# Mephisto405/WCMC

Hardware: AMD Instinct MI355X
Metric: 128x128 MC patches/sec (train step), KPCN-Manifold (higher is better)
Workload: dtype bf16x321h

## Files before the change

### wcmc_amd/csrc/pathnet_fused.hip

```cpp
#include <stdlib.h>

#include "common.h"

namespace wcmc {

typedef __bf16 bf16x8 __attribute__((ext_vector_type(8)));
typedef unsigned short u16;
typedef short s16x4 __attribute__((ext_vector_type(4)));
typedef unsigned u32x2 __attribute__((ext_vector_type(2)));
typedef unsigned u32x4 __attribute__((ext_vector_type(4)));

constexpr unsigned E3_OOB = 0x80000000u;
constexpr int E3_TP = 64;
constexpr int E3_C = 64;
constexpr int E3_RS = 80;
constexpr int E3_TILE = E3_TP * E3_RS;

__device__ __forceinline__ u16 e3_bf(float x) { return __builtin_bit_cast(u16, (__bf16)x); }
__device__ __forceinline__ float e3_f(u16 h) { return __builtin_bit_cast(float, (unsigned)h << 16); }
__device__ __forceinline__ float e3_u2f(unsigned v) { return __builtin_bit_cast(float, v); }
__device__ __forceinline__ unsigned e3_f2u(float v) { return __builtin_bit_cast(unsigned, v); }

struct E3Params {
  const u16* x; int64_t M; int Cp0, Kt0;
// ... 196 lines not shown
                                                                       p.gm ? (int)p.gm_bytes : 0, 0x00020000);
  const E3W w0 = e3_load_w(p.wp0, 16 * ct + fr, q, p.Kt0), w1 = e3_load_w(p.wp1, 16 * ct + fr, q);
  const E3W t2 = e3_load_w(p.wt2, 16 * ct + fr, q), t1 = e3_load_w(p.wt1, 16 * ct + fr, q);
  float b0[4], b1[4];
#pragma unroll
  for (int e = 0; e < 4; ++e) { const int co = 16 * ct + 4 * q + e; b0[e] = p.b0[co]; b1[e] = p.b1[co]; }
  f32x4 g2[2], g1[2], g0[2];
#pragma unroll
  for (int j = 0; j < 2; ++j) { g2[j] = f32x4{0.f, 0.f, 0.f, 0.f}; g1[j] = g2[j]; g0[j] = g2[j]; }
  const int nci0 = (p.Cp0 + 15) >> 4;
  float sb2[4] = {0.f, 0.f, 0.f, 0.f}, sb1[4] = {0.f, 0.f, 0.f, 0.f}, sb0[4] = {0.f, 0.f, 0.f, 0.f};
  const int64_t ntiles = (p.M + E3_TP - 1) / E3_TP;
  const int64_t SHW = (int64_t)p.S * p.HW;

  struct DyPre { u32x4 g[2], m[2]; };
  const bool mean_uniform = p.HW % E3_TP == 0;
  auto load_dy = [&](int64_t m0) {
    DyPre r;
    const unsigned gbase = (unsigned)(m0 * p.gy_ps * 4);
    const int left = (int)(p.M - m0 < E3_TP ? p.M - m0 : E3_TP);
    const int64_t b = m0 / SHW, hw0 = m0 % p.HW;
    const unsigned mbase = (unsigned)((b * p.HW + hw0) * p.gm_ps * 4);
#pragma unroll
    for (int k = 0; k < 2; ++k) {
      const int v = tid + 512 * k, px = v >> 4, c4 = (v & 15) * 4;
      const bool ok = px < left;
      r.g[k] = __builtin_amdgcn_raw_buffer_load_b128(gyr, ok ? gbase + (unsigned)((px * p.gy_ps + c4) * 4) : E3_OOB, 0, 0);
      unsigned moff;
      if (mean_uniform) {
        moff = mbase + (unsigned)((px * p.gm_ps + c4) * 4);
      } else {
        const unsigned m = (unsigned)m0 + (unsigned)px, bi = m / (unsigned)SHW, hw = m % (unsigned)p.HW;
        moff = (bi * (unsigned)p.HW + hw) * (unsigned)(p.gm_ps * 4) + (unsigned)(c4 * 4);
      }
      r.m[k] = __builtin_amdgcn_raw_buffer_load_b128(gmr, (ok && p.gm) ? moff : E3_OOB, 0, 0);
    }
    return r;
  };
  int64_t t = blockIdx.x;
  E3XPre<512> pre;
  DyPre dpre;
  if (t < ntiles) { pre = e3_load_x<512>(xr, t * E3_TP, p.M, p.Cp0, tid); dpre = load_dy(t * E3_TP); }
  for (; t < ntiles; t += gridDim.x) {
    e3_store_x<512>(pre, XH, XL, tid);
#pragma unroll
    for (int k = 0; k < 2; ++k) {
      const int v = tid + 512 * k, px = v >> 4, c4 = (v & 15) * 4;
      u16 hi[4];
#pragma unroll
      for (int e = 0; e < 4; ++e) {
        const float d = e3_u2f(dpre.g[k][e]) + e3_u2f(dpre.m[k][e]) * p.gm_scale;
        sb2[e] += d;
        hi[e] = e3_bf(d);
      }
      *reinterpret_cast<u32x2*>(DYH + px * E3_RS + c4) = u32x2{(unsigned)hi[0] | ((unsigned)hi[1] << 16), (unsigned)hi[2] | ((unsigned)hi[3] << 16)};
    }
    const int64_t tn = t + gridDim.x;
    if (tn < ntiles) { pre = e3_load_x<512>(xr, tn * E3_TP, p.M, p.Cp0, tid); dpre = load_dy(tn * E3_TP); }
    __syncthreads();
    f32x4 acc[2], acca[2];
    unsigned m0bits = 0;
    e3_gemm<3, 2>(acc, w0, XH, XL, pt0, fr, q);
    e3_gemm<2, 2>(acca, t2, DYH, nullptr, pt0, fr, q);
#pragma unroll
    for (int i = 0; i < 2; ++i) {
      u16 hi[4], lo[4];
#pragma unroll
      for (int e = 0; e < 4; ++e) {
        const float t_ = acc[i][e] + b0[e];
        const float v = t_ > 0.f ? t_ : 0.f;
        hi[e] = e3_bf(v);
        lo[e] = e3_bf(v - e3_f(hi[e]));
        m0bits |= (e3_f(hi[e]) > 0.f ? 1u : 0u) << (4 * i + e);
      }
      const int o = (16 * (pt0 + i) + fr) * E3_RS + 16 * ct + 4 * q;
      *reinterpret_cast<u32x2*>(H0H + o) = u32x2{(unsigned)hi[0] | ((unsigned)hi[1] << 16), (unsigned)hi[2] | ((unsigned)hi[3] << 16)};
      *reinterpret_cast<u32x2*>(H0L + o) = u32x2{(unsigned)lo[0] | ((unsigned)lo[1] << 16), (unsigned)lo[2] | ((unsigned)lo[3] << 16)};
    }
    __syncthreads();
    e3_gemm<3, 2>(acc, w1, H0H, H0L, pt0, fr, q);
#pragma unroll
    for (int i = 0; i < 2; ++i) {
      u16 hi[4], dh[4];
#pragma unroll
      for (int e = 0; e < 4; ++e) {
        const float t_ = acc[i][e] + b1[e];
        hi[e] = e3_bf(t_ > 0.f ? t_ : 0.f);
        const float d = e3_f(hi[e]) > 0.f ? acca[i][e] : 0.f;
        sb1[e] += d;
        dh[e] = e3_bf(d);
      }
      const int o = (16 * (pt0 + i) + fr) * E3_RS + 16 * ct + 4 * q;
      *reinterpret_cast<u32x2*>(H1H + o) = u32x2{(unsigned)hi[0] | ((unsigned)hi[1] << 16), (unsigned)hi[2] | ((unsigned)hi[3] << 16)};
      *reinterpret_cast<u32x2*>(DH1H + o) = u32x2{(unsigned)dh[0] | ((unsigned)dh[1] << 16), (unsigned)dh[2] | ((unsigned)dh[3] << 16)};
    }
    __syncthreads();
    e3_gemm<2, 2>(acc, t1, DH1H, nullptr, pt0, fr, q);
#pragma unroll
    for (int i = 0; i < 2; ++i) {
      u16 dh[4];
#pragma unroll
      for (int e = 0; e < 4; ++e) {
        const float d = ((m0bits >> (4 * i + e)) & 1u) ? acc[i][e] : 0.f;
        sb0[e] += d;
        dh[e] = e3_bf(d);
      }
      const int o = (16 * (pt0 + i) + fr) * E3_RS + 16 * ct + 4 * q;
      *reinterpret_cast<u32x2*>(DH0H + o) = u32x2{(unsigned)dh[0] | ((unsigned)dh[1] << 16), (unsigned)dh[2] | ((unsigned)dh[3] << 16)};
    }
    __syncthreads();
#pragma unroll
    for (int kk = 0; kk < 2; ++kk) {
      const bf16x8 a2 = e3_tr(DYH, kk, ct, lane), a1 = e3_tr(DH1H, kk, ct, lane), a0 = e3_tr(DH0H, kk, ct, lane);
#pragma unroll
      for (int jj = 0; jj < 2; ++jj) {
        const int j = pt0 + jj;
        const bf16x8 bh1 = e3_tr(H1H, kk, j, lane), bh0 = e3_tr(H0H, kk, j, lane);
        g2[jj] = __builtin_amdgcn_mfma_f32_16x16x32_bf16(a2, bh1, g2[jj], 0, 0, 0);
        g1[jj] = __builtin_amdgcn_mfma_f32_16x16x32_bf16(a1, bh0, g1[jj], 0, 0, 0);
        if (j < nci0) {
          const bf16x8 bx = e3_tr(XH, kk, j, lane);
          g0[jj] = __builtin_amdgcn_mfma_f32_16x16x32_bf16(a0, bx, g0[jj], 0, 0, 0);
        }
      }
    }
    __syncthreads();
  }
  float* ws = p.ws + (int64_t)blockIdx.x * E3_WS_PER_BLOCK;
#pragma unroll
  for (int jj = 0; jj < 2; ++jj)
#pragma unroll
    for (int e = 0; e < 4; ++e) {
      const int co = 16 * ct + 4 * q + e, j = pt0 + jj, ci = 16 * j + fr;
      ws[(0 * E3_C + co) * E3_C + ci] = g2[jj][e];
      ws[(1 * E3_C + co) * E3_C + ci] = g1[jj][e];
      ws[(2 * E3_C + co) * E3_C + ci] = j < nci0 ? g0[jj][e] : 0.f;
    }
#pragma unroll
  for (int e = 0; e < 4; ++e) {
    red[0][tid >> 4][(tid & 15) * 4 + e] = sb2[e];
    red[1][16 * ph + fr][16 * ct + 4 * q + e] = sb1[e];
    red[2][16 * ph + fr][16 * ct + 4 * q + e] = sb0[e];
  }
  __syncthreads();
  if (tid < 3 * E3_C) {
    const int l = tid / E3_C, c = tid - l * E3_C;
    float s = 0.f;
#pragma unroll
    for (int r = 0; r < 32; ++r) s += red[l][r][c];
    ws[3 * E3_C * E3_C + l * E3_C + c] = s;
  }
}

__global__ __launch_bounds__(256) void embed3_bwd_finish_kernel(const float* __restrict__ ws, int nblk, int Cin0, float* __restrict__ dw0,
                                                                float* __restrict__ db0, float* __restrict__ dw1, float* __restrict__ db1,
                                                                float* __restrict__ dw2, float* __restrict__ db2) {
  const int i = blockIdx.x * 256 + threadIdx.x;
  if (i >= E3_WS_PER_BLOCK) return;
  float a[8] = {0.f, 0.f, 0.f, 0.f, 0.f, 0.f, 0.f, 0.f};
  int b = 0;
  for (; b + 8 <= nblk; b += 8) {
#pragma unroll
    for (int u = 0; u < 8; ++u) a[u] += ws[(int64_t)(b + u) * E3_WS_PER_BLOCK + i];
  }
  for (; b < nblk; ++b) a[0] += ws[(int64_t)b * E3_WS_PER_BLOCK + i];
  const float s = ((a[0] + a[1]) + (a[2] + a[3])) + ((a[4] + a[5]) + (a[6] + a[7]));
  if (i < 3 * E3_C * E3_C) {
    const int l = i / (E3_C * E3_C), r = i - l * E3_C * E3_C, co = r / E3_C, ci = r - co * E3_C;
    if (l == 0) dw2[co * E3_C + ci] = s;
    else if (l == 1) dw1[co * E3_C + ci] = s;
    else if (ci < Cin0) dw0[co * Cin0 + ci] = s;
  } else {
    const int r = i - 3 * E3_C * E3_C, l = r / E3_C, c = r - l * E3_C;
    (l == 0 ? db2 : l == 1 ? db1 : db0)[c] = s;
  }
}

constexpr int F2_C = 128;
constexpr int F2_RS = 144;
constexpr int F2_TILE = E3_TP * F2_RS;
constexpr int F2_ORS = 48;
constexpr int F2_W1RS = 2 * 128 + 8;

struct F2Params {
  const float* y; int y_ps;
  const float* prop; int p_ps;
  int B, S; int64_t HW;
  const u16* wp0; const u16* wp1;
  const float* b0; const float* b1; int outc;
  float* out; int os;
  const u16* wt0; const u16* wt1;
  const float* gout;
  float* dy; float* dprop;
  float* ws;
  unsigned y_bytes, p_bytes, o_bytes, dy_bytes, dp_bytes;
};
constexpr int F2_WS_PER_BLOCK = F2_C * F2_C + 16 * F2_C + F2_C + 16;

struct F2W { bf16x8 h[4], l[4]; };
__device__ __forceinline__ F2W f2_load_w(const u16* wp, int row, int q) {
  F2W w;
#pragma unroll
  for (int c = 0; c < 4; ++c) {
    const u16* a = wp + (int64_t)(row * 2) * F2_C + c * 32 + q * 8;
    w.h[c] = *reinterpret_cast<const bf16x8*>(a);
    w.l[c] = *reinterpret_cast<const bf16x8*>(a + F2_C);
  }
  return w;
}
template <int TERMS, int NPT>
__device__ __forceinline__ void f2_gemm(f32x4 (&acc)[NPT], const F2W& w, const u16* th, const u16* tl, int pt0, int fr, int q) {
#pragma unroll
  for (int i = 0; i < NPT; ++i) {
    acc[i] = f32x4{0.f, 0.f, 0.f, 0.f};
#pragma unroll
    for (int c = 0; c < 4; ++c) {
      const int o = (16 * (pt0 + i) + fr) * F2_RS + c * 32 + q * 8;
      const bf16x8 ah = *reinterpret_cast<const bf16x8*>(th + o);
      acc[i] = __builtin_amdgcn_mfma_f32_16x16x32_bf16(w.l[c], ah, acc[i], 0, 0, 0);
      if (TERMS == 3) {
        const bf16x8 al = *reinterpret_cast<const bf16x8*>(tl + o);
        acc[i] = __builtin_amdgcn_mfma_f32_16x16x32_bf16(w.h[c], al, acc[i], 0, 0, 0);
      }
      acc[i] = __builtin_amdgcn_mfma_f32_16x16x32_bf16(w.h[c], ah, acc[i], 0, 0, 0);
    }
  }
}
__device__ __forceinline__ bf16x8 f2_tr(const u16* tile, int rs, int kk, int ct, int lane) {
  const int g = lane >> 4, li = lane & 15, tq = li >> 2, tp = li & 3;
  const u16* a0 = tile + (kk * 32 + 4 * g + tq) * rs + ct * 16 + 4 * tp;
  const s16x4 lo4 = __builtin_amdgcn_ds_read_tr16_b64_v4i16((s16x4 __attribute__((address_space(3)))*)(a0));
  const s16x4 hi4 = __builtin_amdgcn_ds_read_tr16_b64_v4i16((s16x4 __attribute__((address_space(3)))*)(a0 + 16 * rs));
  typedef short s16x8 __attribute__((ext_vector_type(8)));
  const s16x8 cat = {lo4[0], lo4[1], lo4[2], lo4[3], hi4[0], hi4[1], hi4[2], hi4[3]};
  return __builtin_bit_cast(bf16x8, cat);
}
struct F2Pre { u32x4 v[2]; };
__device__ __forceinline__ F2Pre f2_load64(const __amdgpu_buffer_rsrc_t r, int64_t m0, int ps, int tid) {
  F2Pre o;
  const unsigned base = (unsigned)(m0 * ps * 4);
#pragma unroll
  for (int k = 0; k < 2; ++k) {
    const int v = tid + 512 * k, px = v >> 4, c4 = (v & 15) * 4;
    o.v[k] = __builtin_amdgcn_raw_buffer_load_b128(r, base + (unsigned)((px * ps + c4) * 4), 0, 0);
  }
  return o;
}
__device__ __forceinline__ void f2_store64_split(const F2Pre& o, u16* th, u16* tl, int c0, int tid) {
#pragma unroll
  for (int k = 0; k < 2; ++k) {
    const int v = tid + 512 * k, px = v >> 4, c4 = (v & 15) * 4;
    u16 hi[4], lo[4];
#pragma unroll
    for (int e = 0; e < 4; ++e) {
      const float f = e3_u2f(o.v[k][e]);
      hi[e] = e3_bf(f);
      lo[e] = e3_bf(f - e3_f(hi[e]));
    }
    const int a = px * F2_RS + c0 + c4;
    *reinterpret_cast<u32x2*>(th + a) = u32x2{(unsigned)hi[0] | ((unsigned)hi[1] << 16), (unsigned)hi[2] | ((unsigned)hi[3] << 16)};
    *reinterpret_cast<u32x2*>(tl + a) = u32x2{(unsigned)lo[0] | ((unsigned)lo[1] << 16), (unsigned)lo[2] | ((unsigned)lo[3] << 16)};
  }
}
__device__ __forceinline__ void f2_store_relu_split(const f32x4 (&acc)[4], const float (&b)[4], u16* th, u16* tl, int wave, int fr, int q) {
#pragma unroll
  for (int i = 0; i < 4; ++i) {
    u16 hi[4], lo[4];
#pragma unroll
    for (int e = 0; e < 4; ++e) {
      const float t = acc[i][e] + b[e];
      const float v = t > 0.f ? t : 0.f;
      hi[e] = e3_bf(v);
      lo[e] = e3_bf(v - e3_f(hi[e]));
    }
    const int o = (16 * i + fr) * F2_RS + 16 * wave + 4 * q;
    *reinterpret_cast<u32x2*>(th + o) = u32x2{(unsigned)hi[0] | ((unsigned)hi[1] << 16), (unsigned)hi[2] | ((unsigned)hi[3] << 16)};
    *reinterpret_cast<u32x2*>(tl + o) = u32x2{(unsigned)lo[0] | ((unsigned)lo[1] << 16), (unsigned)lo[2] | ((unsigned)lo[3] << 16)};
  }
}

template <bool BWD>
__global__ __launch_bounds__(512, 1) void final2_kernel(F2Params p) {
  extern __shared__ __attribute__((aligned(16))) u16 lds[];
  u16* const CH = lds; u16* const CL = lds + F2_TILE; u16* const HH = lds + 2 * F2_TILE; u16* const HL = lds + 3 * F2_TILE;
  u16* const DHH = lds + 4 * F2_TILE;
  u16* const DOH = lds + 5 * F2_TILE;
  float* const stg = reinterpret_cast<float*>(HL);
  float* const red = reinterpret_cast<float*>(lds + 5 * F2_TILE + E3_TP * F2_ORS);
  const int tid = threadIdx.x, lane = tid & 63, wave = tid >> 6, fr = lane & 15, q = lane >> 4;
  const __amdgpu_buffer_rsrc_t yr = __builtin_amdgcn_make_buffer_rsrc((void*)p.y, 0, (int)p.y_bytes, 0x00020000);
  const __amdgpu_buffer_rsrc_t pr = __builtin_amdgcn_make_buffer_rsrc((void*)p.prop, 0, (int)p.p_bytes, 0x00020000);
  const __amdgpu_buffer_rsrc_t orr = __builtin_amdgcn_make_buffer_rsrc((void*)(BWD ? (void*)p.gout : (void*)p.out), 0, (int)p.o_bytes, 0x00020000);
  u16* const W1S = reinterpret_cast<u16*>(red + 16 * F2_C + 64 * 8);
  const F2W w0 = f2_load_w(p.wp0, 16 * wave + fr, q);
  F2W w1;
  if (!BWD) w1 = f2_load_w(p.wp1, fr, q);
  float b0[4], b1[4];
#pragma unroll
  for (int e = 0; e < 4; ++e) { b0[e] = p.b0[16 * wave + 4 * q + e]; b1[e] = (4 * q + e < p.outc) ? p.b1[4 * q + e] : 0.f; }
  const int oq = p.os >> 2;
  const int64_t tpi = p.HW / E3_TP;
  const int64_t nsuper = (int64_t)p.B * tpi;

  F2W t0;
  bf16x8 t1h, t1l;
  f32x4 gw0[8], gw1;
  float sb0[4] = {0.f, 0.f, 0.f, 0.f}, sb1[4] = {0.f, 0.f, 0.f, 0.f};
  __amdgpu_buffer_rsrc_t dyr = yr, dpr = yr;
  if (BWD) {
    t0 = f2_load_w(p.wt0, 16 * wave + fr, q);
    const u16* a = p.wt1 + (int64_t)((16 * wave + fr) * 2) * 32 + q * 8;
    t1h = *reinterpret_cast<const bf16x8*>(a); t1l = *reinterpret_cast<const bf16x8*>(a + 32);
#pragma unroll
    for (int j = 0; j < 8; ++j) gw0[j] = f32x4{0.f, 0.f, 0.f, 0.f};
    gw1 = f32x4{0.f, 0.f, 0.f, 0.f};
    dyr = __builtin_amdgcn_make_buffer_rsrc((void*)p.dy, 0, (int)p.dy_bytes, 0x00020000);
    dpr = __builtin_amdgcn_make_buffer_rsrc((void*)p.dprop, 0, (int)p.dp_bytes, 0x00020000);
    for (int i = tid; i < E3_TP * F2_ORS / 2; i += 512) reinterpret_cast<unsigned*>(DOH)[i] = 0u;
    *reinterpret_cast<u32x4*>(W1S + (tid >> 5) * F2_W1RS + (tid & 31) * 8) = *reinterpret_cast<const u32x4*>(p.wp1 + tid * 8);
  }

  for (int64_t st = blockIdx.x; st < nsuper; st += gridDim.x) {
    const int64_t b = st / tpi, hw0 = (st - b * tpi) * E3_TP;
    F2Pre pp = f2_load64(pr, b * p.HW + hw0, p.p_ps, tid);
    F2Pre yp = f2_load64(yr, (b * p.S) * p.HW + hw0, p.y_ps, tid);
    __syncthreads();
    f2_store64_split(pp, CH, CL, 64, tid);
    f32x4 dpacc[4];
#pragma unroll
    for (int i = 0; i < 4; ++i) dpacc[i] = f32x4{0.f, 0.f, 0.f, 0.f};
    for (int s = 0; s < p.S; ++s) {
      const int64_t m0 = (b * p.S + s) * p.HW + hw0;
      f2_store64_split(yp, CH, CL, 0, tid);
      u32x4 go = {0u, 0u, 0u, 0u};
      if (BWD && wave < 4 && q < oq)
        go = __builtin_amdgcn_raw_buffer_load_b128(orr, (unsigned)(m0 * p.os * 4) + (unsigned)((16 * wave + fr) * p.os * 4 + q * 16), 0, 0);
      if (s + 1 < p.S) yp = f2_load64(yr, (b * p.S + s + 1) * p.HW + hw0, p.y_ps, tid);
      __syncthreads();
      f32x4 acc[4];
      f2_gemm<3, 4>(acc, w0, CH, CL, 0, fr, q);
      f2_store_relu_split(acc, b0, HH, HL, wave, fr, q);
      __syncthreads();
      float ov[4] = {0.f, 0.f, 0.f, 0.f};
      if (wave < 4) {
        f32x4 a2[1];
        if (BWD) {
          a2[0] = f32x4{0.f, 0.f, 0.f, 0.f};
#pragma unroll
          for (int c = 0; c < 4; ++c) {
            const int o = (16 * wave + fr) * F2_RS + c * 32 + q * 8;
            const bf16x8 ah = *reinterpret_cast<const bf16x8*>(HH + o), al = *reinterpret_cast<const bf16x8*>(HL + o);
            const bf16x8 wh = *reinterpret_cast<const bf16x8*>(W1S + fr * F2_W1RS + c * 32 + q * 8);
            const bf16x8 wl = *reinterpret_cast<const bf16x8*>(W1S + fr * F2_W1RS + F2_C + c * 32 + q * 8);
            a2[0] = __builtin_amdgcn_mfma_f32_16x16x32_bf16(wl, ah, a2[0], 0, 0, 0);
            a2[0] = __builtin_amdgcn_mfma_f32_16x16x32_bf16(wh, al, a2[0], 0, 0, 0);
            a2[0] = __builtin_amdgcn_mfma_f32_16x16x32_bf16(wh, ah, a2[0], 0, 0, 0);
          }
        } else {
          f2_gemm<3, 1>(a2, w1, HH, HL, wave, fr, q);
        }
#pragma unroll
        for (int e = 0; e < 4; ++e) { const float t = a2[0][e] + b1[e]; ov[e] = (4 * q + e < p.outc && t > 0.f) ? t : 0.f; }
      }
      if (!BWD) {
        if (wave < 4 && q < oq) {
          const u32x4 o4 = {__builtin_bit_cast(unsigned, ov[0]), __builtin_bit_cast(unsigned, ov[1]), __builtin_bit_cast(unsigned, ov[2]),
                            __builtin_bit_cast(unsigned, ov[3])};
          __builtin_amdgcn_raw_buffer_store_b128(o4, orr, (unsigned)(m0 * p.os * 4) + (unsigned)((16 * wave + fr) * p.os * 4 + q * 16), 0, 0);
        }
        __syncthreads();
        continue;
      }
      if (wave < 4 && q < oq) {
        const int px = 16 * wave + fr;
        u16 hi[4];
#pragma unroll
        for (int e = 0; e < 4; ++e) {
          const float d = ov[e] > 0.f ? e3_u2f(go[e]) : 0.f;
          sb1[e] += d;
          hi[e] = e3_bf(d);
        }
        *reinterpret_cast<u32x2*>(DOH + px * F2_ORS + 4 * q) = u32x2{(unsigned)hi[0] | ((unsigned)hi[1] << 16), (unsigned)hi[2] | ((unsigned)hi[3] << 16)};
      }
      __syncthreads();
#pragma unroll
      for (int i = 0; i < 4; ++i) {
        const bf16x8 dof = *reinterpret_cast<const bf16x8*>(DOH + (16 * i + fr) * F2_ORS + q * 8);
        f32x4 a = f32x4{0.f, 0.f, 0.f, 0.f};
        a = __builtin_amdgcn_mfma_f32_16x16x32_bf16(t1l, dof, a, 0, 0, 0);
        a = __builtin_amdgcn_mfma_f32_16x16x32_bf16(t1h, dof, a, 0, 0, 0);
        const int o = (16 * i + fr) * F2_RS + 16 * wave + 4 * q;
        const u32x2 hm = *reinterpret_cast<const u32x2*>(HH + o);
        u16 hi[4];
#pragma unroll
        for (int e = 0; e < 4; ++e) {
          const u16 hv = (u16)((e < 2 ? hm[0] : hm[1]) >> (16 * (e & 1)));
          const float d = e3_f(hv) > 0.f ? a[e] : 0.f;
          sb0[e] += d;
          hi[e] = e3_bf(d);
        }
        *reinterpret_cast<u32x2*>(DHH + o) = u32x2{(unsigned)hi[0] | ((unsigned)hi[1] << 16), (unsigned)hi[2] | ((unsigned)hi[3] << 16)};
      }
      __syncthreads();
      f2_gemm<2, 4>(acc, t0, DHH, nullptr, 0, fr, q);
      if (wave < 4) {
#pragma unroll
        for (int i = 0; i < 4; ++i)
          *reinterpret_cast<float4*>(stg + (16 * i + fr) * 68 + 16 * wave + 4 * q) = make_float4(acc[i][0], acc[i][1], acc[i][2], acc[i][3]);
      } else {
#pragma unroll
        for (int i = 0; i < 4; ++i) dpacc[i] += acc[i];
      }
#pragma unroll
      for (int kk = 0; kk < 2; ++kk) {
        const bf16x8 a0 = f2_tr(DHH, F2_RS, kk, wave, lane);
#pragma unroll
        for (int j = 0; j < 8; ++j) gw0[j] = __builtin_amdgcn_mfma_f32_16x16x32_bf16(a0, f2_tr(CH, F2_RS, kk, j, lane), gw0[j], 0, 0, 0);
        gw1 = __builtin_amdgcn_mfma_f32_16x16x32_bf16(f2_tr(DOH, F2_ORS, kk, 0, lane), f2_tr(HH, F2_RS, kk, wave, lane), gw1, 0, 0, 0);
      }
      __syncthreads();
#pragma unroll
      for (int k = 0; k < 2; ++k) {
        const int v = tid + 512 * k, px = v >> 4, c4 = (v & 15) * 4;
        const float4 o = *reinterpret_cast<const float4*>(stg + px * 68 + c4);
        const u32x4 o4 = {__builtin_bit_cast(unsigned, o.x), __builtin_bit_cast(unsigned, o.y), __builtin_bit_cast(unsigned, o.z),
                          __builtin_bit_cast(unsigned, o.w)};
        __builtin_amdgcn_raw_buffer_store_b128(o4, dyr, (unsigned)(m0 * 256) + (unsigned)(px * 256 + c4 * 4), 0, 0);
      }
    }
    if (BWD && wave >= 4) {
#pragma unroll
      for (int i = 0; i < 4; ++i) {
        const u32x4 o4 = {e3_f2u(dpacc[i][0]), e3_f2u(dpacc[i][1]), e3_f2u(dpacc[i][2]), e3_f2u(dpacc[i][3])};
        __builtin_amdgcn_raw_buffer_store_b128(o4, dpr, (unsigned)((b * p.HW + hw0) * 256) + (unsigned)((16 * i + fr) * 256 + (16 * (wave - 4) + 4 * q) * 4), 0, 0);
      }
    }
  }
  if (!BWD) return;
  float* ws = p.ws + (int64_t)blockIdx.x * F2_WS_PER_BLOCK;
#pragma unroll
  for (int j = 0; j < 8; ++j)
#pragma unroll
    for (int e = 0; e < 4; ++e) ws[(16 * wave + 4 * q + e) * F2_C + 16 * j + fr] = gw0[j][e];
#pragma unroll
  for (int e = 0; e < 4; ++e) ws[F2_C * F2_C + (4 * q + e) * F2_C + 16 * wave + fr] = gw1[e];
  __syncthreads();
  float* redb = red;
#pragma unroll
  for (int e = 0; e < 4; ++e) redb[fr * F2_C + 16 * wave + 4 * q + e] = sb0[e];
  if (wave < 4 && q < 2) {
#pragma unroll
    for (int e = 0; e < 4; ++e) redb[16 * F2_C + (16 * wave + fr) * 8 + 4 * q + e] = sb1[e];
  }
  __syncthreads();
  if (tid < F2_C) {
    float sacc = 0.f;
#pragma unroll
    for (int r = 0; r < 16; ++r) sacc += redb[r * F2_C + tid];
    ws[F2_C * F2_C + 16 * F2_C + tid] = sacc;
  } else if (tid < F2_C + 16) {
    const int c = tid - F2_C;
    float sacc = 0.f;
    if (c < 8)
      for (int r = 0; r < 64; ++r) sacc += redb[16 * F2_C + r * 8 + c];
    ws[F2_C * F2_C + 16 * F2_C + F2_C + c] = sacc;
  }
}

__global__ __launch_bounds__(256) void final2_bwd_finish_kernel(const float* __restrict__ ws, int nblk, int outc, float* __restrict__ dw0,
                                                                float* __restrict__ db0, float* __restrict__ dw1, float* __restrict__ db1) {
  const int i = blockIdx.x * 256 + threadIdx.x;
  if (i >= F2_WS_PER_BLOCK) return;
  float a[8] = {0.f, 0.f, 0.f, 0.f, 0.f, 0.f, 0.f, 0.f};
  int b = 0;
  for (; b + 8 <= nblk; b += 8) {
#pragma unroll
    for (int u = 0; u < 8; ++u) a[u] += ws[(int64_t)(b + u) * F2_WS_PER_BLOCK + i];
  }
  for (; b < nblk; ++b) a[0] += ws[(int64_t)b * F2_WS_PER_BLOCK + i];
  const float s = ((a[0] + a[1]) + (a[2] + a[3])) + ((a[4] + a[5]) + (a[6] + a[7]));
  if (i < F2_C * F2_C) dw0[i] = s;
  else if (i < F2_C * F2_C + 16 * F2_C) {
    const int r = i - F2_C * F2_C, co = r / F2_C, ci = r - co * F2_C;
    if (co < outc) dw1[co * F2_C + ci] = s;
  } else if (i < F2_C * F2_C + 16 * F2_C + F2_C) db0[i - F2_C * F2_C - 16 * F2_C] = s;
  else {
    const int c = i - F2_C * F2_C - 16 * F2_C - F2_C;
    if (c < outc) db1[c] = s;
  }
}

constexpr int F2W_RS = 2 * F2_C + 8;

__device__ __forceinline__ void f2w_split8(const u32x4 a, const u32x4 b, bf16x8& hi, bf16x8& lo) {
  typedef __bf16 xb2 __attribute__((ext_vector_type(2)));
  typedef float xf2 __attribute__((ext_vector_type(2)));
  unsigned h[4], l[4];
#pragma unroll
  for (int d = 0; d < 4; ++d) {
    const unsigned u0 = d < 2 ? a[2 * d] : b[2 * d - 4], u1 = d < 2 ? a[2 * d + 1] : b[2 * d - 3];
    const xf2 v = {e3_u2f(u0), e3_u2f(u1)};
    h[d] = __builtin_bit_cast(unsigned, __builtin_convertvector(v, xb2));
    const xf2 back = {e3_u2f(h[d] << 16), e3_u2f(h[d] & 0xffff0000u)};
    l[d] = __builtin_bit_cast(unsigned, __builtin_convertvector(v - back, xb2));
  }
  hi = __builtin_bit_cast(bf16x8, u32x4{h[0], h[1], h[2], h[3]});
  lo = __builtin_bit_cast(bf16x8, u32x4{l[0], l[1], l[2], l[3]});
}

template <int NI>
__global__ __launch_bounds__(512, NI == 1 ? 4 : 2) void final2w_fwd_kernel(F2Params p) {
  extern __shared__ __attribute__((aligned(16))) u16 lds[];
  u16* const W0S = lds;
  u16* const W1S = lds + F2_C * F2W_RS;
  float* const B0S = reinterpret_cast<float*>(W1S + 16 * F2W_RS);
  const int tid = threadIdx.x, lane = tid & 63, wave = __builtin_amdgcn_readfirstlane(tid >> 6), fr = lane & 15, q = lane >> 4;
  for (int v = tid; v < F2_C * 32; v += 512)
    *reinterpret_cast<u32x4*>(W0S + (v >> 5) * F2W_RS + (v & 31) * 8) = *reinterpret_cast<const u32x4*>(p.wp0 + (int64_t)v * 8);
  *reinterpret_cast<u32x4*>(W1S + (tid >> 5) * F2W_RS + (tid & 31) * 8) = *reinterpret_cast<const u32x4*>(p.wp1 + tid * 8);
  if (tid < F2_C) B0S[tid] = p.b0[tid];
  __syncthreads();
  const __amdgpu_buffer_rsrc_t yr = __builtin_amdgcn_make_buffer_rsrc((void*)p.y, 0, (int)p.y_bytes, 0x00020000);
  const __amdgpu_buffer_rsrc_t pr = __builtin_amdgcn_make_buffer_rsrc((void*)p.prop, 0, (int)p.p_bytes, 0x00020000);
  const __amdgpu_buffer_rsrc_t orr = __builtin_amdgcn_make_buffer_rsrc((void*)p.out, 0, (int)p.o_bytes, 0x00020000);
  float b1[4];
#pragma unroll
  for (int e = 0; e < 4; ++e) b1[e] = (4 * q + e < p.outc) ? p.b1[4 * q + e] : 0.f;
  const int oq = p.os >> 2;
  const int64_t tpi = p.HW / (16 * NI), nunits = (int64_t)p.B * tpi;
  const int nwaves = (int)gridDim.x * 8;
  auto load8 = [&](const __amdgpu_buffer_rsrc_t r, unsigned base, int ps, int i, int cs, u32x4& a, u32x4& b) {
    const unsigned off = base + (unsigned)(((16 * i + fr) * ps + 32 * cs + 8 * q) * 4);
    a = __builtin_amdgcn_raw_buffer_load_b128(r, off, 0, 0);
    b = __builtin_amdgcn_raw_buffer_load_b128(r, off + 16, 0, 0);
  };
  for (int64_t u = (int64_t)blockIdx.x * 8 + wave; u < nunits; u += nwaves) {
    const int64_t b = u / tpi, hw0 = (u - b * tpi) * (16 * NI);
    bf16x8 ph[NI][2], pl[NI][2];
    {
      const unsigned base = (unsigned)((b * p.HW + hw0) * p.p_ps * 4);
#pragma unroll
      for (int i = 0; i < NI; ++i)
#pragma unroll
        for (int cs = 0; cs < 2; ++cs) {
          u32x4 a, c;
          load8(pr, base, p.p_ps, i, cs, a, c);
          f2w_split8(a, c, ph[i][cs], pl[i][cs]);
        }
    }
    u32x4 ya[NI][2], yb[NI][2];
    {
      const unsigned base = (unsigned)(((b * p.S) * p.HW + hw0) * p.y_ps * 4);
#pragma unroll
      for (int i = 0; i < NI; ++i)
#pragma unroll
        for (int cs = 0; cs < 2; ++cs) load8(yr, base, p.y_ps, i, cs, ya[i][cs], yb[i][cs]);
    }
    for (int s = 0; s < p.S; ++s) {
      const int64_t m0 = (b * p.S + s) * p.HW + hw0;
      bf16x8 yh[NI][2], yl[NI][2];
#pragma unroll
      for (int i = 0; i < NI; ++i)
#pragma unroll
        for (int cs = 0; cs < 2; ++cs) f2w_split8(ya[i][cs], yb[i][cs], yh[i][cs], yl[i][cs]);
      if (s + 1 < p.S) {
        const unsigned base = (unsigned)((m0 + p.HW) * p.y_ps * 4);
#pragma unroll
        for (int i = 0; i < NI; ++i)
#pragma unroll
          for (int cs = 0; cs < 2; ++cs) load8(yr, base, p.y_ps, i, cs, ya[i][cs], yb[i][cs]);
      }
      f32x4 a2[NI];
#pragma unroll
      for (int i = 0; i < NI; ++i) a2[i] = f32x4{0.f, 0.f, 0.f, 0.f};
      int wrow = fr * F2W_RS + q * 8;
      asm volatile("" : "+v"(wrow));
#pragma unroll
      for (int s2 = 0; s2 < 4; ++s2) {
        f32x4 acc[2][NI];
#pragma unroll
        for (int jj = 0; jj < 2; ++jj) {
          const int j = 2 * s2 + jj;
          #pragma unroll
          for (int i = 0; i < NI; ++i) acc[jj][i] = f32x4{0.f, 0.f, 0.f, 0.f};
#pragma unroll
          for (int c = 0; c < 4; ++c) {
            const u16* wa = W0S + wrow + 16 * j * F2W_RS + c * 32;
            const bf16x8 wh = *reinterpret_cast<const bf16x8*>(wa), wl = *reinterpret_cast<const bf16x8*>(wa + F2_C);
#pragma unroll
            for (int i = 0; i < NI; ++i) {
              const bf16x8 ah = c < 2 ? yh[i][c & 1] : ph[i][c & 1], al = c < 2 ? yl[i][c & 1] : pl[i][c & 1];
              acc[jj][i] = __builtin_amdgcn_mfma_f32_16x16x32_bf16(wl, ah, acc[jj][i], 0, 0, 0);
              acc[jj][i] = __builtin_amdgcn_mfma_f32_16x16x32_bf16(wh, al, acc[jj][i], 0, 0, 0);
              acc[jj][i] = __builtin_amdgcn_mfma_f32_16x16x32_bf16(wh, ah, acc[jj][i], 0, 0, 0);
            }
          }
        }
        const f32x4 bA = *reinterpret_cast<const f32x4*>(B0S + 32 * s2 + 4 * q), bB = *reinterpret_cast<const f32x4*>(B0S + 32 * s2 + 16 + 4 * q);
        const u16* w1a = W1S + wrow - 4 * q + 32 * s2;
        const u32x2 h0 = *reinterpret_cast<const u32x2*>(w1a), h1 = *reinterpret_cast<const u32x2*>(w1a + 16);
        const u32x2 l0 = *reinterpret_cast<const u32x2*>(w1a + F2_C), l1 = *reinterpret_cast<const u32x2*>(w1a + F2_C + 16);
        const bf16x8 w1h = __builtin_bit_cast(bf16x8, u32x4{h0[0], h0[1], h1[0], h1[1]});
        const bf16x8 w1l = __builtin_bit_cast(bf16x8, u32x4{l0[0], l0[1], l1[0], l1[1]});
#pragma unroll
        for (int i = 0; i < NI; ++i) {
          u32x4 ra, rb;
#pragma unroll
          for (int e = 0; e < 4; ++e) {
            const float tA = acc[0][i][e] + bA[e], tB = acc[1][i][e] + bB[e];
            ra[e] = e3_f2u(tA > 0.f ? tA : 0.f);
            rb[e] = e3_f2u(tB > 0.f ? tB : 0.f);
          }
          bf16x8 hh, hl;
          f2w_split8(ra, rb, hh, hl);
          a2[i] = __builtin_amdgcn_mfma_f32_16x16x32_bf16(w1l, hh, a2[i], 0, 0, 0);
          a2[i] = __builtin_amdgcn_mfma_f32_16x16x32_bf16(w1h, hl, a2[i], 0, 0, 0);
          a2[i] = __builtin_amdgcn_mfma_f32_16x16x32_bf16(w1h, hh, a2[i], 0, 0, 0);
        }
      }
      if (q < oq) {
#pragma unroll
        for (int i = 0; i < NI; ++i) {
          u32x4 o4;
#pragma unroll
          for (int e = 0; e < 4; ++e) { const float t = a2[i][e] + b1[e]; o4[e] = e3_f2u((4 * q + e < p.outc && t > 0.f) ? t : 0.f); }
          __builtin_amdgcn_raw_buffer_store_b128(o4, orr, (unsigned)(m0 * p.os * 4) + (unsigned)((16 * i + fr) * p.os * 4 + q * 16), 0, 0);
        }
      }
    }
  }
}
constexpr size_t F2W_LDS_FWD = (size_t)(F2_C + 16) * F2W_RS * sizeof(u16) + (size_t)F2_C * sizeof(float);

static int f2_grid() { return 256; }
constexpr size_t F2_LDS_FWD = (size_t)4 * F2_TILE * sizeof(u16);
constexpr size_t F2_LDS_BWD = (size_t)5 * F2_TILE * sizeof(u16) + (size_t)E3_TP * F2_ORS * sizeof(u16) + (size_t)(16 * F2_C + 64 * 8) * sizeof(float) +
                              (size_t)16 * F2_W1RS * sizeof(u16);

static int e3_grid_bwd() { return 256; }

}

using namespace wcmc;

extern "C" int wcmc_embed3_supported(int Cin, int C1, int C2, int C3) {
  return Cin >= 1 && Cin <= 64 && C1 == 64 && C2 == 64 && C3 == 64;
}

extern "C" size_t wcmc_embed3_bwd_workspace_bytes(void) { return (size_t)e3_grid_bwd() * E3_WS_PER_BLOCK * sizeof(float); }

static int e3_fill(E3Params& p, const void* x_split, int64_t M, int Cin, const void* wp0, const float* b0, const void* wp1,
                   const float* b1) {
  WCMC_REQUIRE(x_split && wp0 && wp1 && b0 && b1 && M > 0 && Cin >= 1 && Cin <= 64, WCMC_ERR_BAD_ARG, "embed3: bad argument");
  WCMC_REQUIRE(aligned16(x_split) && aligned16(wp0) && aligned16(wp1), WCMC_ERR_ALIGNMENT, "embed3: buffers must be 16-byte aligned");
  p.x = (const u16*)x_split; p.M = M; p.Cp0 = round_up(Cin, 8); p.Kt0 = round_up(p.Cp0, 32);
  p.wp0 = (const u16*)wp0; p.wp1 = (const u16*)wp1; p.b0 = b0; p.b1 = b1;
  const int64_t xb = M * 4 * p.Cp0, yb = M * 256;
  WCMC_REQUIRE(xb < 0x7ff00000ll && yb < 0x7ff00000ll, WCMC_ERR_BAD_ARG, "embed3: more than 2 GiB per tensor (split the batch)");
  p.x_bytes = (unsigned)xb; p.y_bytes = (unsigned)yb;
  return 0;
}

extern "C" int wcmc_embed3_fwd(const void* x_split, int64_t M, int Cin, const void* wp0, const float* b0, const void* wp1,
                               const float* b1, const void* wp2, const float* b2, float* y, void* stream) {
  E3Params p = {};
  if (int rc = e3_fill(p, x_split, M, Cin, wp0, b0, wp1, b1)) return rc;
  WCMC_REQUIRE(wp2 && b2 && y && aligned16(wp2) && aligned16(y), WCMC_ERR_BAD_ARG, "embed3_fwd: bad argument");
  p.wp2 = (const u16*)wp2; p.b2 = b2; p.y = y;
  const int64_t ntiles = (M + E3_TP - 1) / E3_TP;
  const unsigned grid = (unsigned)(ntiles < 768 ? ntiles : 768);
  hipLaunchKernelGGL(embed3_fwd_kernel<false>, dim3(grid), dim3(256), 0, (hipStream_t)stream, p);
  return check_launch("embed3_fwd");
}

extern "C" int wcmc_embed3_mean_supported(int S, int64_t HW) { return S >= 1 && HW > 0 && HW % E3_TP == 0; }

extern "C" int wcmc_embed3_mean_fwd(const void* x_split, int64_t M, int Cin, const void* wp0, const float* b0, const void* wp1,
                                    const float* b1, const void* wp2, const float* b2, float* y, float* y_mean, int S, int64_t HW,
                                    void* stream) {
  E3Params p = {};
  if (int rc = e3_fill(p, x_split, M, Cin, wp0, b0, wp1, b1)) return rc;
  WCMC_REQUIRE(wp2 && b2 && y && y_mean && aligned16(wp2) && aligned16(y) && aligned16(y_mean), WCMC_ERR_BAD_ARG, "embed3_mean_fwd: bad argument");
  WCMC_REQUIRE(wcmc_embed3_mean_supported(S, HW) && M % ((int64_t)S * HW) == 0, WCMC_ERR_BAD_ARG,
               "embed3_mean_fwd: M must be B * S * HW with HW a multiple of 64 (ask wcmc_embed3_mean_supported)");
  p.wp2 = (const u16*)wp2; p.b2 = b2; p.y = y; p.ym = y_mean; p.ym_bytes = (unsigned)((M / S) * 256);
  p.S = S; p.HW = HW; p.gm_scale = 1.0f / (float)S;
  const int64_t nsuper = M / ((int64_t)S * E3_TP);
  const unsigned grid = (unsigned)(nsuper < 768 ? nsuper : 768);
  hipLaunchKernelGGL(embed3_fwd_kernel<true>, dim3(grid), dim3(256), 0, (hipStream_t)stream, p);
  return check_launch("embed3_mean_fwd");
}

extern "C" int wcmc_embed3_bwd(const void* x_split, int64_t M, int Cin, const void* wp0, const float* b0, const void* wp1,
                               const float* b1, const void* wt1, const void* wt2, const float* gy, int gy_pixel_stride,
                               const float* gm, int gm_pixel_stride, int S, int64_t HW, float gm_scale, float* dw0, float* db0, float* dw1, float* db1, float* dw2, float* db2,
                               void* workspace, size_t workspace_bytes, void* stream) {
  E3Params p = {};
  if (int rc = e3_fill(p, x_split, M, Cin, wp0, b0, wp1, b1)) return rc;
  WCMC_REQUIRE(wt1 && wt2 && (gy || gm) && dw0 && db0 && dw1 && db1 && dw2 && db2 && workspace && aligned16(wt1) && aligned16(wt2) &&
                   (!gy || aligned16(gy)) && (!gm || aligned16(gm)) && aligned16(workspace),
               WCMC_ERR_BAD_ARG, "embed3_bwd: bad argument");
  WCMC_REQUIRE(workspace_bytes >= wcmc_embed3_bwd_workspace_bytes(), WCMC_ERR_WORKSPACE, "embed3_bwd: workspace too small");
  WCMC_REQUIRE(!gm || (S >= 1 && HW >= 1 && M % ((int64_t)S * HW) == 0), WCMC_ERR_BAD_ARG,
               "embed3_bwd: with the gradient of the spp mean M must be B * S * HW");
  p.wt1 = (const u16*)wt1; p.wt2 = (const u16*)wt2; p.gy = gy; p.gm = gm; p.S = S > 0 ? S : 1; p.HW = HW > 0 ? HW : M;
  p.gm_scale = gm_scale; p.ws = (float*)workspace;
  WCMC_REQUIRE((!gy || (gy_pixel_stride >= 64 && gy_pixel_stride % 4 == 0)) && (!gm || (gm_pixel_stride >= 64 && gm_pixel_stride % 4 == 0)),
               WCMC_ERR_ALIGNMENT, "embed3_bwd: pixel strides must be multiples of 4 floats and >= 64");
  p.gy_ps = gy ? gy_pixel_stride : 64; p.gm_ps = gm ? gm_pixel_stride : 64;
  const int64_t gyb = gy ? ((M - 1) * p.gy_ps + 64) * 4 : 0, gmb = gm ? ((M / p.S - 1) * p.gm_ps + 64) * 4 : 0;
  WCMC_REQUIRE(gyb < 0x7ff00000ll && gmb < 0x7ff00000ll, WCMC_ERR_BAD_ARG, "embed3_bwd: gradient view spans more than 2 GiB");
  p.gy_bytes = (unsigned)gyb; p.gm_bytes = (unsigned)gmb;
  const int nblk = e3_grid_bwd();
  hipLaunchKernelGGL(embed3_bwd_kernel, dim3((unsigned)nblk), dim3(512), 0, (hipStream_t)stream, p);
  if (int rc = check_launch("embed3_bwd")) return rc;
  hipLaunchKernelGGL(embed3_bwd_finish_kernel, dim3((unsigned)((E3_WS_PER_BLOCK + 255) / 256)), dim3(256), 0, (hipStream_t)stream,
                     (const float*)workspace, nblk, Cin, dw0, db0, dw1, db1, dw2, db2);
  return check_launch("embed3_bwd_finish");
}


extern "C" int wcmc_final2_supported(int C1, int C2, int Chid, int outc, int64_t HW) {
  return C1 == 64 && C2 == 64 && Chid == 128 && outc >= 1 && outc <= 8 && HW > 0 && HW % 64 == 0;
}
extern "C" size_t wcmc_final2_bwd_workspace_bytes(void) { return (size_t)f2_grid() * F2_WS_PER_BLOCK * sizeof(float); }

static int f2_fill(F2Params& p, const float* y, int y_ps, const float* prop, int p_ps, int B, int S, int64_t HW, const void* wp0,
                   const float* b0, const void* wp1, const float* b1, int outc) {
  WCMC_REQUIRE(y && prop && wp0 && wp1 && b0 && b1 && B > 0 && S > 0 && wcmc_final2_supported(64, 64, 128, outc, HW), WCMC_ERR_BAD_ARG,
               "final2: bad argument (64 + 64 -> 128 -> <= 8 channels, H*W a multiple of 64)");
  WCMC_REQUIRE(aligned16(y) && aligned16(prop) && aligned16(wp0) && aligned16(wp1) && y_ps >= 64 && y_ps % 4 == 0 && p_ps >= 64 && p_ps % 4 == 0,
               WCMC_ERR_ALIGNMENT, "final2: views must be 16-byte aligned with pixel strides that are multiples of 4 floats");
  p.y = y; p.y_ps = y_ps; p.prop = prop; p.p_ps = p_ps; p.B = B; p.S = S; p.HW = HW;
  p.wp0 = (const u16*)wp0; p.wp1 = (const u16*)wp1; p.b0 = b0; p.b1 = b1; p.outc = outc; p.os = outc <= 4 ? 4 : 8;
  const int64_t M = (int64_t)B * S * HW;
  const int64_t yb = ((M - 1) * y_ps + 64) * 4, pb = (((int64_t)B * HW - 1) * p_ps + 64) * 4, ob = M * p.os * 4;
  WCMC_REQUIRE(yb < 0x7ff00000ll && pb < 0x7ff00000ll && M * 256 < 0x7ff00000ll, WCMC_ERR_BAD_ARG, "final2: more than 2 GiB per tensor");
// ... 54 lines not shown
```

Measured before the change: 729.2.

## Hoist prop-branch backward GEMMs out of per-sample loop via summed gradients

The gradient with respect to the per-pixel property inputs is linear in the hidden-layer gradient, and those inputs are shared across samples. So the kernel now accumulates the hidden gradient over samples in registers and runs the prop-input GEMMs once per tile, using a hi/lo bf16 split of the sum. The weight-gradient columns for those inputs get the same treatment. The per-sample dy GEMM is split across all 8 waves by row halves instead of 4 waves doing all rows. This removes per-sample MFMA work and trades it for extra register accumulators, one extra synchronisation and a small change in rounding order.

```diff
diff --git a/wcmc_amd/csrc/pathnet_fused.hip b/wcmc_amd/csrc/pathnet_fused.hip
--- a/wcmc_amd/csrc/pathnet_fused.hip
+++ b/wcmc_amd/csrc/pathnet_fused.hip
@@ -522,13 +522,14 @@
   const int64_t tpi = p.HW / E3_TP;
   const int64_t nsuper = (int64_t)p.B * tpi;
 
+  const int ct = wave & 3, ph = wave >> 2;
   F2W t0;
   bf16x8 t1h, t1l;
   f32x4 gw0[8], gw1;
   float sb0[4] = {0.f, 0.f, 0.f, 0.f}, sb1[4] = {0.f, 0.f, 0.f, 0.f};
   __amdgpu_buffer_rsrc_t dyr = yr, dpr = yr;
   if (BWD) {
-    t0 = f2_load_w(p.wt0, 16 * wave + fr, q);
+    t0 = f2_load_w(p.wt0, 16 * ct + fr, q);
     const u16* a = p.wt1 + (int64_t)((16 * wave + fr) * 2) * 32 + q * 8;
     t1h = *reinterpret_cast<const bf16x8*>(a); t1l = *reinterpret_cast<const bf16x8*>(a + 32);
 #pragma unroll
@@ -546,9 +547,9 @@
     F2Pre yp = f2_load64(yr, (b * p.S) * p.HW + hw0, p.y_ps, tid);
     __syncthreads();
     f2_store64_split(pp, CH, CL, 64, tid);
-    f32x4 dpacc[4];
-#pragma unroll
-    for (int i = 0; i < 4; ++i) dpacc[i] = f32x4{0.f, 0.f, 0.f, 0.f};
+    f32x4 D[4];
+#pragma unroll
+    for (int i = 0; i < 4; ++i) D[i] = f32x4{0.f, 0.f, 0.f, 0.f};
     for (int s = 0; s < p.S; ++s) {
       const int64_t m0 = (b * p.S + s) * p.HW + hw0;
       f2_store64_split(yp, CH, CL, 0, tid);
@@ -618,24 +619,21 @@
           const float d = e3_f(hv) > 0.f ? a[e] : 0.f;
           sb0[e] += d;
           hi[e] = e3_bf(d);
+          D[i][e] += e3_f(hi[e]);
         }
         *reinterpret_cast<u32x2*>(DHH + o) = u32x2{(unsigned)hi[0] | ((unsigned)hi[1] << 16), (unsigned)hi[2] | ((unsigned)hi[3] << 16)};
       }
       __syncthreads();
-      f2_gemm<2, 4>(acc, t0, DHH, nullptr, 0, fr, q);
-      if (wave < 4) {
-#pragma unroll
-        for (int i = 0; i < 4; ++i)
-          *reinterpret_cast<float4*>(stg + (16 * i + fr) * 68 + 16 * wave + 4 * q) = make_float4(acc[i][0], acc[i][1], acc[i][2], acc[i][3]);
-      } else {
-#pragma unroll
-        for (int i = 0; i < 4; ++i) dpacc[i] += acc[i];
-      }
+      f32x4 dya[2];
+      f2_gemm<2, 2>(dya, t0, DHH, nullptr, 2 * ph, fr, q);
+#pragma unroll
+      for (int i = 0; i < 2; ++i)
+        *reinterpret_cast<float4*>(stg + (16 * (2 * ph + i) + fr) * 68 + 16 * ct + 4 * q) = make_float4(dya[i][0], dya[i][1], dya[i][2], dya[i][3]);
 #pragma unroll
       for (int kk = 0; kk < 2; ++kk) {
         const bf16x8 a0 = f2_tr(DHH, F2_RS, kk, wave, lane);
 #pragma unroll
-        for (int j = 0; j < 8; ++j) gw0[j] = __builtin_amdgcn_mfma_f32_16x16x32_bf16(a0, f2_tr(CH, F2_RS, kk, j, lane), gw0[j], 0, 0, 0);
+        for (int j = 0; j < 4; ++j) gw0[j] = __builtin_amdgcn_mfma_f32_16x16x32_bf16(a0, f2_tr(CH, F2_RS, kk, j, lane), gw0[j], 0, 0, 0);
         gw1 = __builtin_amdgcn_mfma_f32_16x16x32_bf16(f2_tr(DOH, F2_ORS, kk, 0, lane), f2_tr(HH, F2_RS, kk, wave, lane), gw1, 0, 0, 0);
       }
       __syncthreads();
@@ -648,11 +646,45 @@
         __builtin_amdgcn_raw_buffer_store_b128(o4, dyr, (unsigned)(m0 * 256) + (unsigned)(px * 256 + c4 * 4), 0, 0);
       }
     }
-    if (BWD && wave >= 4) {
+    if (BWD) {
+      const F2W tp = f2_load_w(p.wt0, 64 + 16 * ct + fr, q);
 #pragma unroll
       for (int i = 0; i < 4; ++i) {
-        const u32x4 o4 = {e3_f2u(dpacc[i][0]), e3_f2u(dpacc[i][1]), e3_f2u(dpacc[i][2]), e3_f2u(dpacc[i][3])};
-        __builtin_amdgcn_raw_buffer_store_b128(o4, dpr, (unsigned)((b * p.HW + hw0) * 256) + (unsigned)((16 * i + fr) * 256 + (16 * (wave - 4) + 4 * q) * 4), 0, 0);
+        u16 hi[4], lo[4];
+#pragma unroll
+        for (int e = 0; e < 4; ++e) {
+          hi[e] = e3_bf(D[i][e]);
+          lo[e] = e3_bf(D[i][e] - e3_f(hi[e]));
+        }
+        const int o = (16 * i + fr) * F2_RS + 16 * wave + 4 * q;
+        *reinterpret_cast<u32x2*>(DHH + o) = u32x2{(unsigned)hi[0] | ((unsigned)hi[1] << 16), (unsigned)hi[2] | ((unsigned)hi[3] << 16)};
+        *reinterpret_cast<u32x2*>(HH + o) = u32x2{(unsigned)lo[0] | ((unsigned)lo[1] << 16), (unsigned)lo[2] | ((unsigned)lo[3] << 16)};
+      }
+      __syncthreads();
+#pragma unroll
+      for (int i = 0; i < 2; ++i) {
+        f32x4 a = f32x4{0.f, 0.f, 0.f, 0.f};
+#pragma unroll
+        for (int c = 0; c < 4; ++c) {
+          const int o = (16 * (2 * ph + i) + fr) * F2_RS + c * 32 + q * 8;
+          const bf16x8 dhi = *reinterpret_cast<const bf16x8*>(DHH + o), dlo = *reinterpret_cast<const bf16x8*>(HH + o);
+          a = __builtin_amdgcn_mfma_f32_16x16x32_bf16(tp.l[c], dlo, a, 0, 0, 0);
+          a = __builtin_amdgcn_mfma_f32_16x16x32_bf16(tp.h[c], dlo, a, 0, 0, 0);
+          a = __builtin_amdgcn_mfma_f32_16x16x32_bf16(tp.l[c], dhi, a, 0, 0, 0);
+          a = __builtin_amdgcn_mfma_f32_16x16x32_bf16(tp.h[c], dhi, a, 0, 0, 0);
+        }
+        const u32x4 o4 = {e3_f2u(a[0]), e3_f2u(a[1]), e3_f2u(a[2]), e3_f2u(a[3])};
+        __builtin_amdgcn_raw_buffer_store_b128(o4, dpr, (unsigned)((b * p.HW + hw0) * 256) + (unsigned)((16 * (2 * ph + i) + fr) * 256 + (16 * ct + 4 * q) * 4), 0, 0);
+      }
+#pragma unroll
+      for (int kk = 0; kk < 2; ++kk) {
+        const bf16x8 alo = f2_tr(HH, F2_RS, kk, wave, lane), ahi = f2_tr(DHH, F2_RS, kk, wave, lane);
+#pragma unroll
+        for (int j = 4; j < 8; ++j) {
+          const bf16x8 cp = f2_tr(CH, F2_RS, kk, j, lane);
+          gw0[j] = __builtin_amdgcn_mfma_f32_16x16x32_bf16(alo, cp, gw0[j], 0, 0, 0);
+          gw0[j] = __builtin_amdgcn_mfma_f32_16x16x32_bf16(ahi, cp, gw0[j], 0, 0, 0);
+        }
       }
     }
   }
```

Result: faster. 738.2 (median of 6 runs) (+1.2%).
